# NNU-GISA/MetricSfM

Hardware: AMD Instinct MI355X
Metric: BA iterations/sec (higher is better)
Workload: dtype f64; 1 GPU; BASELINE config 3: 500 cameras / 200000 points / 1200000 observations, dense-Schur LM, Huber(1); reduced_system_order=3003, parallelism=points sharded over 1 rank(s), camera block all-reduced, collective=none (1 rank), successful_steps=2789, unsuccessful_steps=0

## Files before the change

metricsfm_amd/csrc/ba.hip:

```cpp
#include <algorithm>
#include <array>
#include <chrono>
#include <cmath>
#include <cstdlib>
#include <cstring>
#include <functional>

#include <rocprim/rocprim.hpp>

#include "ba_device.h"
#include "ba_partials.h"
#include "common.h"
#include "solve_riders.h"


#define PSTRIDE 80
#define CHUNK 1024
#define FTF_CHUNK 512
static int chunk_for(long total, int max_chunk) {
  const long c = 64 * ((total / 1024 + 63) / 64);
  return (int)std::max<long>(64, std::min<long>(max_chunk, c));
}
#define F_JCJC 0
#define F_JMJC 36
#define F_JMJM 54
#define F_JCR 63
#define F_JMR 69
#define F_TU 72
static_assert(PSTRIDE == MODELSUM_PSTRIDE && F_JMJM == MODELSUM_JMJM && F_JMR == MODELSUM_JMR, "solve_riders.h reads the FTF partials");

enum { S_COST = 0, S_MCC, S_DX2, S_X2, S_FAIL, S_XCOST, S_GMAX, S_RANK0 = 8, S_N = 64 };

struct BaPtrs {
  int A, AE, ncb, nmb, npb, NCR;
  const double *cam, *model, *pt;
  const double* rot;
  const int *o_cam, *o_model, *o_pt, *o_cb, *o_mb, *o_pb, *o_cpos, *o_pm;
  const double *o_x, *o_y, *o_w;
  double *lin_r, *lin_Jc, *lin_Jm;
  const double *scale_c, *scale_m, *scale_p;
  double huber;
};

__device__ __forceinline__ double linearize_core(const double (&pose)[6], const double (&rc)[4], const double (&cm)[3], const double (&X)[3], double ox,
                                                 double oy, double ow, const double (&sc)[6], const double (&sm)[3], const double (&sp)[3], double huber,
                                                 double& r0, double& r1, double (&jc)[12], double (&jm)[6], double (&jp)[6]) {
  double r[2], J[24];
  msfm_reproj(pose, rc, cm, X, ox, oy, ow, r, J);
  double rho0, rho1;
  msfm_huber(huber, r[0] * r[0] + r[1] * r[1], rho0, rho1);
  const double sq = sqrt(rho1);
  r0 = sq * r[0]; r1 = sq * r[1];
#pragma unroll
  for (int j = 0; j < 6; j++) {
    const double s = sq * sc[j];
    jc[j] = s * J[j];
    jc[6 + j] = s * J[12 + j];
  }
#pragma unroll
  for (int j = 0; j < 3; j++) {
    const double s = sq * sm[j];
    jm[j] = s * J[6 + j];
    jm[3 + j] = s * J[12 + 6 + j];
    const double spj = sq * sp[j];
    jp[j] = spj * J[9 + j];
    jp[3 + j] = spj * J[12 + 9 + j];
  }
  return 0.5 * rho0;
}
__device__ __forceinline__ double obs_linearize(const BaPtrs& P, int i, double& r0, double& r1, double (&jc)[12], double (&jm)[6], double (&jp)[6]) {
  const int c = P.o_cam[i], m = P.o_model[i], p = P.o_pt[i];
  const int cb = P.o_cb[i], mb = P.o_mb[i], pb = P.o_pb[i];
  double pose[6], rc[4], cm[3], X[3];
#pragma unroll
  for (int j = 0; j < 6; j++) pose[j] = P.cam[6 * (size_t)c + j];
#pragma unroll
  for (int j = 0; j < 4; j++) rc[j] = P.rot[4 * (size_t)c + j];
#pragma unroll
  for (int j = 0; j < 3; j++) { cm[j] = P.model[3 * (size_t)m + j]; X[j] = P.pt[3 * (size_t)p + j]; }
  const double ox = P.o_x[i], oy = P.o_y[i], ow = P.o_w[i];
  double r[2], J[24];
  msfm_reproj(pose, rc, cm, X, ox, oy, ow, r, J);
  __builtin_amdgcn_sched_barrier(0);
  double sc[6], sm[3], sp[3];
#pragma unroll
  for (int j = 0; j < 6; j++) sc[j] = cb >= 0 ? P.scale_c[6 * cb + j] : 0.0;
#pragma unroll
  for (int j = 0; j < 3; j++) { sm[j] = mb >= 0 ? P.scale_m[3 * mb + j] : 0.0; sp[j] = pb >= 0 ? P.scale_p[3 * (size_t)pb + j] : 0.0; }
  double rho0, rho1;
  msfm_huber(P.huber, r[0] * r[0] + r[1] * r[1], rho0, rho1);
  const double sq = sqrt(rho1);
  r0 = sq * r[0]; r1 = sq * r[1];
#pragma unroll
  for (int j = 0; j < 6; j++) {
    const double s = sq * sc[j];
    jc[j] = s * J[j];
    jc[6 + j] = s * J[12 + j];
  }
#pragma unroll
  for (int j = 0; j < 3; j++) {
    const double s = sq * sm[j];
    jm[j] = s * J[6 + j];
    jm[3 + j] = s * J[12 + 6 + j];
    const double spj = sq * sp[j];
    jp[j] = spj * J[9 + j];
    jp[3 + j] = spj * J[12 + 9 + j];
  }
  return 0.5 * rho0;
}
template <bool WRITE_JAC>
__device__ __forceinline__ void linearize_block(const BaPtrs& P, int i0, int blk, double* __restrict__ cost_partial, double* sh) {
  const int i = i0 + blk * 256 + threadIdx.x;
  double cost = 0.0;
  if (i < P.A) {
    if (WRITE_JAC) {
      double r0, r1, jc[12], jm[6], jp[6];
      cost = obs_linearize(P, i, r0, r1, jc, jm, jp);
      const size_t nt = (size_t)(P.A - P.AE), it = (size_t)(i - P.AE);
      P.lin_r[it] = r0;
      P.lin_r[nt + it] = r1;
#pragma unroll
      for (int j = 0; j < 12; j++) P.lin_Jc[(size_t)j * nt + it] = jc[j];
#pragma unroll
      for (int j = 0; j < 6; j++) P.lin_Jm[(size_t)j * nt + it] = jm[j];
    } else {
      const int c = P.o_cam[i], m = P.o_model[i], p = P.o_pt[i];
      double pose[6], rc[4], cm[3], X[3];
#pragma unroll
      for (int j = 0; j < 6; j++) pose[j] = P.cam[6 * (size_t)c + j];
#pragma unroll
      for (int j = 0; j < 4; j++) rc[j] = P.rot[4 * (size_t)c + j];
#pragma unroll
      for (int j = 0; j < 3; j++) { cm[j] = P.model[3 * (size_t)m + j]; X[j] = P.pt[3 * (size_t)p + j]; }
      double r[2];
      msfm_reproj(pose, rc, cm, X, P.o_x[i], P.o_y[i], P.o_w[i], r, nullptr);
      double rho0, rho1;
      msfm_huber(P.huber, r[0] * r[0] + r[1] * r[1], rho0, rho1);
      cost = 0.5 * rho0;
    }
  }
  const double t = block_sum256(cost, sh);
  if (threadIdx.x == 0) cost_partial[blk] = t;
}
template <bool WRITE_JAC>
__global__ __launch_bounds__(256) void k_linearize(BaPtrs P, int i0, double* __restrict__ cost_partial, const double* __restrict__ spec = nullptr) {
  __shared__ double sh[4];
  if (spec && spec[0] == 0.0) return;
  linearize_block<WRITE_JAC>(P, i0, blockIdx.x, cost_partial, sh);
}

__global__ __launch_bounds__(256) void k_rot_cache(int Nc, const double* __restrict__ cam, double* __restrict__ rot) {
  const int c = blockIdx.x * 256 + threadIdx.x;
  if (c < Nc) msfm_rot_prepare(cam + 6 * (size_t)c, rot + 4 * (size_t)c);
}

template <bool WRITE_JAC>
__device__ __forceinline__ void gps_block(int blk, int ncb, const int* __restrict__ cb_cam, const double* __restrict__ cam,
                                          const double* __restrict__ gps, double w, double huber,
                                          const double* __restrict__ scale_c, double* __restrict__ g_r,
                                          double* __restrict__ g_J, double* __restrict__ cost_partial, double* sh) {
  const int cb = blk * 256 + threadIdx.x;
  double cost = 0.0;
  if (cb < ncb) {
    const int c = cb_cam[cb];
    const double wz[3] = {w, w, w / 5.0};
    double r[3], J[3], s = 0.0;
#pragma unroll
    for (int k = 0; k < 3; k++) {
      const double d = cam[6 * (size_t)c + 3 + k] - gps[3 * (size_t)cb + k];
      r[k] = wz[k] * fabs(d);
      J[k] = wz[k] * (d < 0.0 ? -1.0 : 1.0);
      s += r[k] * r[k];
    }
    double rho0, rho1;
    msfm_huber(huber, s, rho0, rho1);
    cost = 0.5 * rho0;
    if (WRITE_JAC) {
      const double sq = sqrt(rho1);
#pragma unroll
      for (int k = 0; k < 3; k++) {
        g_r[3 * (size_t)cb + k] = sq * r[k];
        g_J[3 * (size_t)cb + k] = sq * J[k] * scale_c[6 * cb + 3 + k];
      }
    }
  }
  const double t = block_sum256(cost, sh);
  if (threadIdx.x == 0) cost_partial[blk] = t;
}
template <bool WRITE_JAC>
__global__ __launch_bounds__(256) void k_gps(int ncb, const int* __restrict__ cb_cam, const double* __restrict__ cam,
                                              const double* __restrict__ gps, double w, double huber,
                                              const double* __restrict__ scale_c, double* __restrict__ g_r,
                                              double* __restrict__ g_J, double* __restrict__ cost_partial, const double* __restrict__ spec = nullptr) {
  __shared__ double sh[4];
  if (spec && spec[0] == 0.0) return;
  gps_block<WRITE_JAC>(blockIdx.x, ncb, cb_cam, cam, gps, w, huber, scale_c, g_r, g_J, cost_partial, sh);
}

struct ReduceJobs {
  int count;
  struct { const double* p; int n; int slot; int is_max; } job[6];
  const int* fail;
  int fail_slot;
};
__global__ __launch_bounds__(1024) void k_reduce(ReduceJobs J, double* __restrict__ scal) {
  __shared__ double sh[16];
  const double* __restrict__ partial = J.job[blockIdx.x].p;
  const int n = J.job[blockIdx.x].n, slot = J.job[blockIdx.x].slot, is_max = J.job[blockIdx.x].is_max;
  double v0 = 0.0, v1 = 0.0, v2 = 0.0, v3 = 0.0;
  int i = threadIdx.x;
  for (; i + 3072 < n; i += 4096) {
    const double a = partial[i], b = partial[i + 1024], c = partial[i + 2048], d = partial[i + 3072];
    if (is_max) { v0 = fmax(v0, a); v1 = fmax(v1, b); v2 = fmax(v2, c); v3 = fmax(v3, d); }
    else { v0 += a; v1 += b; v2 += c; v3 += d; }
  }
  for (; i < n; i += 1024) v0 = is_max ? fmax(v0, partial[i]) : v0 + partial[i];
  double v = is_max ? fmax(fmax(v0, v1), fmax(v2, v3)) : (v0 + v1) + (v2 + v3);
  v = is_max ? wave_max(v) : wave_sum(v);
  if ((threadIdx.x & 63) == 0) sh[threadIdx.x >> 6] = v;
  __syncthreads();
  if (threadIdx.x == 0) {
    double t = sh[0];
// ... 901 lines not shown
#pragma unroll
    for (int k = 0; k < 9; k++) if (k == lane) v = -acc[k];
    if (rb == cbk && lead) {
      v += modelsum[12 * (size_t)rb + lane];
      if (a == c) { const double q = sqrt(diag_m[3 * rb + a] / radius); v += q * q; }
    }
    M[(size_t)(mo + 3 * rb + a) * ld + mo + 3 * cbk + c] = v;
  } else if (lane < 12 && rb == cbk) {
    const int a = lane - 9;
    double u = 0.0;
#pragma unroll
    for (int k = 9; k < 12; k++) if (k == lane) u = acc[k];
    M[(size_t)n * ld + mo + 3 * rb + a] = (lead ? modelsum[12 * (size_t)rb + 9 + a] : 0.0) - u;
  }
}

__device__ __forceinline__ void asm_rhs_cam(int i, int ncb, const double* __restrict__ camftf, const int* __restrict__ cb_off,
                                            double* __restrict__ M, int ld, int n, int lead) {
  if (i >= 6 * ncb) return;
  const int cb = i / 6, a = i % 6;
  const double* f = camftf + (size_t)cb * PSTRIDE;
  M[(size_t)n * ld + cb_off[cb] + a] = lead ? f[F_JCR + a] - f[F_TU + a] : 0.0;
}

struct AsmArgs {
  int n_cc, n_mc, n_mm, n_rhs, n_padcol;
  const int* padcol;
  const int* cc_fold_first;
  const uint8_t* cc_live;
  const double* cc_fold_partial;
  const int* mc_fold_range;
  const double* mc_fold_partial;
  const int *cc_row, *cc_col, *cc_first, *mc_row, *mc_col, *mc_first, *mm_row, *mm_col, *mm_first, *cb_mb, *cb_off;
  const double *cc_partial, *mc_partial, *mm_partial, *camftf, *diag_c, *modelsum, *diag_m;
  double radius;
  int ncb, mo, n, ld, lead;
  double* M;
};
__global__ __launch_bounds__(64) void k_asm_all(AsmArgs a) {
  int b = blockIdx.x;
  if (b < a.n_cc) {
    const int sub = (int)threadIdx.x / 18;
    asm_cc(b, sub, (int)threadIdx.x - 18 * sub, a.cc_row, a.cc_col, a.cc_first, a.cc_live, a.cc_partial, a.cc_fold_first, a.cc_fold_partial, a.camftf, a.diag_c, a.radius, a.cb_off, a.M, a.ld, a.lead);
    return;
  }
  b -= a.n_cc;
  if (b < a.n_mc) { asm_mc(b, a.mc_row, a.mc_col, a.mc_first, a.mc_partial, a.mc_fold_range, a.mc_fold_partial, a.camftf, a.cb_mb, a.cb_off, a.mo, a.M, a.ld, a.lead); return; }
  b -= a.n_mc;
  if (b < a.n_mm) { asm_mm(b, a.mm_row, a.mm_col, a.mm_first, a.mm_partial, a.modelsum, a.diag_m, a.radius, a.mo, a.n, a.M, a.ld, a.lead); return; }
  b -= a.n_mm;
  if (b < a.n_rhs) { asm_rhs_cam(b * 64 + (int)threadIdx.x, a.ncb, a.camftf, a.cb_off, a.M, a.ld, a.n, a.lead); return; }
  b -= a.n_rhs;
  const int i = b * 64 + (int)threadIdx.x;
  if (i < a.n_padcol) a.M[(size_t)a.padcol[i] * a.ld + a.padcol[i]] = 1.0;
}

__global__ void k_pad_diag(int npadcol, const int* __restrict__ padcol, double* __restrict__ M, int ld) {
  const int i = blockIdx.x * blockDim.x + threadIdx.x;
  if (i < npadcol) M[(size_t)padcol[i] * ld + padcol[i]] = 1.0;
}

__global__ __launch_bounds__(256) void k_copy3(size_t n0, const double* __restrict__ a0, double* __restrict__ b0, size_t n1,
                                               const double* __restrict__ a1, double* __restrict__ b1, size_t n2,
                                               const double* __restrict__ a2, double* __restrict__ b2) {
  const size_t i = (size_t)blockIdx.x * 256 + threadIdx.x;
  if (i < n0) b0[i] = a0[i];
  if (i < n1) b1[i] = a1[i];
  if (i < n2) b2[i] = a2[i];
}


__global__ void k_scale_scal(double* __restrict__ scal, int slot, double f) { scal[slot] *= f; }

__global__ __launch_bounds__(256) void k_update_params(int ncb, int nmb, const int* __restrict__ cb_cam, const int* __restrict__ mb_model,
                                                        const int* __restrict__ cb_off, int mo, const double* __restrict__ zsys,
                                                        const double* __restrict__ scale_c, const double* __restrict__ scale_m,
                                                        const double* __restrict__ cam, double* __restrict__ cam_c,
                                                        const double* __restrict__ model, double* __restrict__ model_c, double* __restrict__ z,
                                                        int* __restrict__ fail, double* __restrict__ dx2_partial, double* __restrict__ x2_partial,
                                                        double count_weight) {
  __shared__ double sh[4];
  const int i = blockIdx.x * 256 + threadIdx.x;
  double dx2 = 0.0, x2 = 0.0;
  if (i < 6 * ncb + 3 * nmb) {
    double zv, sc, xv;
    double* dst;
    if (i < 6 * ncb) {
      const int b = i / 6, a = i % 6;
      zv = zsys[cb_off[b] + a];
      sc = scale_c[i];
      const size_t k = (size_t)cb_cam[b] * 6 + a;
      xv = cam[k];
      dst = cam_c + k;
    } else {
      const int j = i - 6 * ncb, b = j / 3, a = j % 3;
      zv = zsys[mo + j];
      sc = scale_m[j];
      const size_t k = (size_t)mb_model[b] * 3 + a;
      xv = model[k];
      dst = model_c + k;
    }
    z[i] = zv;
    if (!isfinite(zv)) atomicOr(fail, 4);
    const double cand = xv + (-zv) * sc;
    *dst = cand;
    const double d = cand - xv;
    dx2 = d * d * count_weight;
    x2 = xv * xv * count_weight;
  }
  const double t1 = block_sum256(dx2, sh);
  const double t2 = block_sum256(x2, sh);
  if (threadIdx.x == 0) { dx2_partial[blockIdx.x] = t1; x2_partial[blockIdx.x] = t2; }
}
__global__ void k_col_map(int ncb, int nmb, const int* __restrict__ cb_cam, const int* __restrict__ mb_model, const int* __restrict__ cb_off,
                          int mo, int* __restrict__ col_param, int* __restrict__ col_slot) {
  const int i = blockIdx.x * 256 + threadIdx.x;
  if (i >= 6 * ncb + 3 * nmb) return;
  int col, slot;
  if (i < 6 * ncb) { const int b = i / 6, a = i % 6; col = cb_off[b] + a; slot = cb_cam[b] * 6 + a; }
  else { const int j = i - 6 * ncb, b = j / 3, a = j % 3; col = mo + j; slot = mb_model[b] * 3 + a; }
  col_param[col] = i;
  col_slot[col] = slot;
}
__device__ __forceinline__ void update_block_sums(int n, const double* __restrict__ dx2s, const double* __restrict__ x2s,
                                                  double* __restrict__ dx2_partial, double* __restrict__ x2_partial, double* sh) {
  const int i = blockIdx.x * 256 + threadIdx.x;
  double dx2 = 0.0, x2 = 0.0;
  if (i < n) { dx2 = dx2s[i]; x2 = x2s[i]; }
  const double t1 = block_sum256(dx2, sh);
  const double t2 = block_sum256(x2, sh);
  if (threadIdx.x == 0) { dx2_partial[blockIdx.x] = t1; x2_partial[blockIdx.x] = t2; }
}

struct BackPtrs {
  BaPtrs B;
  PtMap map;
  int npb, ncb;
  const int *pt_first, *pb_pt;
  const double *ptL, *z;
  double* pt_c;
  double* cm_Xc;
  int Nc;
  const double* cam_c;
  double* rot_c;
};
struct UpdateSums {
  int nbu, n;
  const double *dx2, *x2;
  double *dx2_partial, *x2_partial;
};

template <int LPP>
__device__ __forceinline__ void k_backsub_body(const BackPtrs& P, double* __restrict__ mcc_partial, double* __restrict__ dx2_partial,
                                               double* __restrict__ x2_partial, double* sh) {
  constexpr int GW = LPP ? LPP : 8;
  const int tid = threadIdx.x, sub = tid & (GW - 1);
  const int pb = ptmap_wg_first(P.map, blockIdx.x) + tid / GW;
  const bool act = pb < ptmap_wg_end(P.map, blockIdx.x);
  for (int c = blockIdx.x * 256 + tid; c < P.Nc; c += gridDim.x * 256) msfm_rot_prepare(P.cam_c + 6 * (size_t)c, P.rot_c + 4 * (size_t)c);
  int f = 0, l = 0;
  if (act) { f = P.pt_first[pb]; l = P.pt_first[pb + 1]; }
  double V00 = 0, V10 = 0, V11 = 0, V20 = 0, V21 = 0, V22 = 0, g0 = 0, g1 = 0, g2 = 0, h0 = 0, h1 = 0, h2 = 0, qr = 0, qq = 0;
  const int n_rounds = LPP ? 1 : (l - f + 7) >> 3;
  for (int rd = 0; rd < n_rounds; rd++) {
    const int i = f + GW * rd + sub;
    if (i < l) {
      double jp[6], r0, r1, q0, q1;
      {
        const int cb = P.B.o_cb[i], mb = P.B.o_mb[i];
        double jc[12], jm[6], zc[6], zm[3];
        obs_linearize(P.B, i, r0, r1, jc, jm, jp);
        __builtin_amdgcn_sched_barrier(0);
        const double* zcp = P.z + 6 * (cb >= 0 ? cb : 0);
        const double* zmp = P.z + 6 * P.ncb + 3 * (mb >= 0 ? mb : 0);
#pragma unroll
        for (int j = 0; j < 6; j++) zc[j] = zcp[j];
#pragma unroll
        for (int j = 0; j < 3; j++) zm[j] = zmp[j];
        q0 = 0.0; q1 = 0.0;
#pragma unroll
        for (int j = 0; j < 6; j++) { q0 -= jc[j] * zc[j]; q1 -= jc[6 + j] * zc[j]; }
#pragma unroll
        for (int j = 0; j < 3; j++) { q0 -= jm[j] * zm[j]; q1 -= jm[3 + j] * zm[j]; }
      }
      const double a0 = jp[0], a1 = jp[1], a2 = jp[2], b0 = jp[3], b1 = jp[4], b2 = jp[5];
      V00 += a0 * a0 + b0 * b0; V10 += a1 * a0 + b1 * b0; V11 += a1 * a1 + b1 * b1;
      V20 += a2 * a0 + b2 * b0; V21 += a2 * a1 + b2 * b1; V22 += a2 * a2 + b2 * b2;
      g0 += a0 * r0 + b0 * r1; g1 += a1 * r0 + b1 * r1; g2 += a2 * r0 + b2 * r1;
      h0 += a0 * q0 + b0 * q1; h1 += a1 * q0 + b1 * q1; h2 += a2 * q0 + b2 * q1;
      qr += q0 * r0 + q1 * r1;
      qq += q0 * q0 + q1 * q1;
    }
  }
  GROUP_SUM(V00) GROUP_SUM(V10) GROUP_SUM(V11) GROUP_SUM(V20) GROUP_SUM(V21) GROUP_SUM(V22)
  GROUP_SUM(g0) GROUP_SUM(g1) GROUP_SUM(g2) GROUP_SUM(h0) GROUP_SUM(h1) GROUP_SUM(h2) GROUP_SUM(qr) GROUP_SUM(qq)
  double mcc = 0.0, dx2 = 0.0, x2 = 0.0, cand0 = 0.0, cand1 = 0.0, cand2 = 0.0;
  if (act && sub == 0) {
    const double* L = P.ptL + 6 * (size_t)pb;
    const double i00 = L[0], l10 = L[1], i11 = L[2], l20 = L[3], l21 = L[4], i22 = L[5];
    double q0 = (g0 + h0) * i00;
    double q1 = ((g1 + h1) - l10 * q0) * i11;
    double q2 = ((g2 + h2) - l20 * q0 - l21 * q1) * i22;
    q2 = q2 * i22;
    q1 = (q1 - l21 * q2) * i11;
    q0 = (q0 - l10 * q1 - l20 * q2) * i00;
    const double s0 = -q0, s1 = -q1, s2 = -q2;
    const double* sc = P.B.scale_p + 3 * (size_t)pb;
    const size_t p = P.pb_pt[pb];
    const double x0 = P.B.pt[3 * p], x1 = P.B.pt[3 * p + 1], x2v = P.B.pt[3 * p + 2];
    const double c0 = x0 + s0 * sc[0], c1 = x1 + s1 * sc[1], c2 = x2v + s2 * sc[2];
    P.pt_c[3 * p] = c0; P.pt_c[3 * p + 1] = c1; P.pt_c[3 * p + 2] = c2;
    cand0 = c0; cand1 = c1; cand2 = c2;
    dx2 = (c0 - x0) * (c0 - x0) + (c1 - x1) * (c1 - x1) + (c2 - x2v) * (c2 - x2v);
    x2 = x0 * x0 + x1 * x1 + x2v * x2v;
    const double sVs = s0 * (V00 * s0 + 2.0 * (V10 * s1 + V20 * s2)) + s1 * (V11 * s1 + 2.0 * V21 * s2) + s2 * V22 * s2;
    mcc = -((s0 * g0 + s1 * g1 + s2 * g2) + qr + 0.5 * sVs + (s0 * h0 + s1 * h1 + s2 * h2) + 0.5 * qq);
  }
  cand0 = __shfl(cand0, 0, GW); cand1 = __shfl(cand1, 0, GW); cand2 = __shfl(cand2, 0, GW);
  for (int rd = 0; rd < n_rounds; rd++) {
    const int i = f + GW * rd + sub;
    if (i < l) {
      const int cp = P.B.o_cpos[i];
      if (cp >= 0) { double* xr = P.cm_Xc + 3 * (size_t)cp; xr[0] = cand0; xr[1] = cand1; xr[2] = cand2; }
    }
  }
  const double t0 = block_sum256(mcc, sh);
  const double t1 = block_sum256(dx2, sh);
  const double t2 = block_sum256(x2, sh);
  if (threadIdx.x == 0) { mcc_partial[blockIdx.x] = t0; dx2_partial[blockIdx.x] = t1; x2_partial[blockIdx.x] = t2; }
}
__global__ __launch_bounds__(256) __attribute__((amdgpu_waves_per_eu(3, 3))) void k_backsub(BackPtrs P, double* __restrict__ mcc_partial, double* __restrict__ dx2_partial,
                                                  double* __restrict__ x2_partial, UpdateSums U) {
  __shared__ double sh[4];
  const int lanes = ptmap_lanes(P.map, blockIdx.x);
  if (lanes == 4) k_backsub_body<4>(P, mcc_partial, dx2_partial, x2_partial, sh);
  else if (lanes == 8) k_backsub_body<8>(P, mcc_partial, dx2_partial, x2_partial, sh);
  else if (lanes == 16) k_backsub_body<16>(P, mcc_partial, dx2_partial, x2_partial, sh);
  else k_backsub_body<0>(P, mcc_partial, dx2_partial, x2_partial, sh);
  if ((int)blockIdx.x < U.nbu) update_block_sums(U.n, U.dx2, U.x2, U.dx2_partial, U.x2_partial, sh);
}

__device__ __forceinline__ void mcc_rest_block(int blk, int A, int AE, int ncb, const int* __restrict__ o_cb, const int* __restrict__ o_mb,
                                               const double* __restrict__ lin_r, const double* __restrict__ lin_Jc,
                                               const double* __restrict__ lin_Jm, const double* __restrict__ z, int has_gps,
                                               const double* __restrict__ g_r, const double* __restrict__ g_J,
                                               double* __restrict__ mcc_partial, double* sh) {
  const int t = blk * 256 + threadIdx.x;
  const int nrest = A - AE;
  double mcc = 0.0;
  if (t < nrest) {
    const int i = AE + t;
    const size_t As = (size_t)nrest, it = (size_t)t;
    double m0 = 0, m1 = 0;
    const int cb = o_cb[i], mb = o_mb[i];
    if (cb >= 0)
      for (int j = 0; j < 6; j++) { const double sj = -z[6 * cb + j]; m0 += lin_Jc[(size_t)j * As + it] * sj; m1 += lin_Jc[(size_t)(6 + j) * As + it] * sj; }
    if (mb >= 0)
      for (int j = 0; j < 3; j++) { const double sj = -z[6 * ncb + 3 * mb + j]; m0 += lin_Jm[(size_t)j * As + it] * sj; m1 += lin_Jm[(size_t)(3 + j) * As + it] * sj; }
    mcc -= m0 * (lin_r[it] + m0 / 2.0) + m1 * (lin_r[As + it] + m1 / 2.0);
  } else if (has_gps && t < nrest + ncb) {
    const int cb = t - nrest;
    for (int k = 0; k < 3; k++) {
      const double m = g_J[3 * (size_t)cb + k] * (-z[6 * cb + 3 + k]);
      mcc -= m * (g_r[3 * (size_t)cb + k] + m / 2.0);
    }
  }
  const double s = block_sum256(mcc, sh);
  if (threadIdx.x == 0) mcc_partial[blk] = s;
}

struct TailArgs {
  int n_zero; double* M; int ld; ZeroMap Z;
  int n_mcc, n_cost, n_gps;
  int A, AE, ncb; const int *o_cb, *o_mb; const double *lin_r, *lin_Jc, *lin_Jm, *z; int has_gps; const double *g_r, *g_J; double* mcc_partial;
  BaPtrs P; double* cost_partial;
  const int* cb_cam; const double *cam_c, *gps; double gps_weight, huber; const double* scale_c; double *g_r_w, *g_J_w;
};
__global__ __launch_bounds__(256) void k_tail(TailArgs a) {
  __shared__ double sh[4];
  int b = blockIdx.x;
  if (b < a.n_zero) { zero_tile_body(b, a.M, a.ld, a.Z); return; }
  b -= a.n_zero;
  if (b < a.n_mcc) { mcc_rest_block(b, a.A, a.AE, a.ncb, a.o_cb, a.o_mb, a.lin_r, a.lin_Jc, a.lin_Jm, a.z, a.has_gps, a.g_r, a.g_J, a.mcc_partial, sh); return; }
  b -= a.n_mcc;
  if (b < a.n_cost) { linearize_block<false>(a.P, 0, b, a.cost_partial, sh); return; }
  b -= a.n_cost;
  gps_block<false>(b, a.ncb, a.cb_cam, a.cam_c, a.gps, a.gps_weight, a.huber, a.scale_c, a.g_r_w, a.g_J_w, a.cost_partial + a.n_cost, sh);
}

__global__ void k_zero_int(int* p) { *p = 0; }
enum { LM_NONE = 0, LM_INVALID, LM_PARAM_TOL, LM_FUNC_TOL, LM_ACCEPT, LM_REJECT };
enum { H_SEQ = 16, H_CODE = 17, H_RADIUS = 18 };
struct LmDecide {
  int on;
  int fresh;
  double x_cost, radius;
  double min_relative_decrease, parameter_tolerance, function_tolerance, max_radius, min_radius;
};
__device__ __forceinline__ double cube_rn(double t) {
  const double h = t * t, l = fma(t, t, -h);
  const double p = h * t, e = fma(h, t, -p);
  return p + fma(l, t, e);
}
__global__ __launch_bounds__(64) void k_publish_scalars(const double* __restrict__ scal, double* h_scal, unsigned long long seq, int* fail, LmDecide D,
                                                        double* __restrict__ spec) {
  const int lane = threadIdx.x;
  if (lane < 16) __hip_atomic_store(&h_scal[lane], scal[lane], __ATOMIC_RELAXED, __HIP_MEMORY_SCOPE_SYSTEM);
  if (lane == 0) {
    int code = LM_NONE;
    double rnew = D.radius;
    if (D.on) {
      const double mcc = scal[S_MCC], cand = scal[S_COST], dx2 = scal[S_DX2], x2 = scal[S_X2];
      const double xc = D.fresh ? scal[S_XCOST] : D.x_cost;
      const bool solved = (int)scal[S_FAIL] == 0;
      if (!(solved && mcc > 0.0)) code = LM_INVALID;
      else if (sqrt(dx2) <= D.parameter_tolerance * (sqrt(x2) + D.parameter_tolerance)) code = LM_PARAM_TOL;
      else if (fabs(xc - cand) <= D.function_tolerance * xc) code = LM_FUNC_TOL;
      else {
        const double rho = (xc - cand) / mcc;
        if (rho > D.min_relative_decrease) {
          code = LM_ACCEPT;
          rnew = D.radius / fmax(1.0 / 3.0, 1.0 - cube_rn(2.0 * rho - 1.0));
          rnew = fmin(D.max_radius, rnew);
        } else code = LM_REJECT;
      }
    }
    spec[0] = (code == LM_ACCEPT && rnew > D.min_radius) ? 1.0 : 0.0;
    spec[1] = rnew;
    __hip_atomic_store(&h_scal[H_CODE], (double)code, __ATOMIC_RELAXED, __HIP_MEMORY_SCOPE_SYSTEM);
    __hip_atomic_store(&h_scal[H_RADIUS], rnew, __ATOMIC_RELAXED, __HIP_MEMORY_SCOPE_SYSTEM);
  }
  __threadfence_system();
  if (lane == 0) {
    __hip_atomic_store(reinterpret_cast<unsigned long long*>(h_scal + H_SEQ), seq, __ATOMIC_RELEASE, __HIP_MEMORY_SCOPE_SYSTEM);
    if (fail) *fail = 0;
  }
}
__global__ void k_fill(int n, double v, double* __restrict__ p) {
  const int i = blockIdx.x * 256 + threadIdx.x;
  if (i < n) p[i] = v;
}

template <bool PACK>
__global__ __launch_bounds__(256) void k_pack_blocks(int nblk, const int* __restrict__ u_row, const int* __restrict__ u_col,
                                                      const int* __restrict__ cb_off, double* __restrict__ M, int ld,
                                                      double* __restrict__ pack) {
  const int e = blockIdx.x * 256 + threadIdx.x;
  if (e >= nblk * 36) return;
  const int b = e / 36, t = e - 36 * b;
  const size_t at = (size_t)(cb_off[u_row[b]] + t / 6) * ld + cb_off[u_col[b]] + t % 6;
  if (PACK) pack[e] = M[at];
  else M[at] = pack[e];
}

struct FoldTables {
  bool on = false;
  bool all = false;
  int n_live = 0;
  DevBuf<int> live_chunk;
  int n_wg = 0, n_slots = 0, n_entries = 0, n_pass = 0;
  DevBuf<int> wg_fold, wg_pass_first, slot_rank, blk_range;
  DevBuf<uint8_t> blk_live;
  DevBuf<FoldPass> pass;
  DevBuf<unsigned> stream;
  DevBuf<double> partial;
  bool mc_on = false, mc_all = false;
  int n_diag = 0, mc_n_live = 0;
  long long mc_entries_folded = 0;
  DevBuf<int> mc_range, mc_live_chunk;
  DevBuf<double> mc_partial;
};

struct PairJobs {
  int n_pairs = 0, n_chunks = 0, n_blocks = 0;
  DevBuf<int> pa, pb, ch_start, ch_end, blk_row, blk_col, blk_chunk_first;
  DevBuf<double> partial;
  std::vector<int> h_row, h_col;
};

struct msfm_ba {
  msfm_ctx* ctx = nullptr;
  msfm_env env;
  int world_at_create = 1;
  double setup_ms = 0;
  int Nc = 0, Nm = 0, Np = 0;
  int ncb = 0, nmb = 0, npb = 0, nred = 0, npad = 0;
  PtMap map = {0, 0, 0, 0, 0, 0, 0};
  int n_short4 = 0;
  int nsys = 0, mo = 0, n_padcol = 0;
  msfm_chol_plan plan;
  int A = 0, AE = 0, NCR = 0, NPM = 0;
// ... 2627 lines not shown
```

metricsfm_amd/csrc/ba_device.h:

```cpp
#pragma once
#include <hip/hip_runtime.h>

__device__ __forceinline__ void msfm_rot_prepare(const double* __restrict__ pose, double* __restrict__ rc) {
  const double a0 = pose[0], a1 = pose[1], a2 = pose[2];
  const double theta2 = a0 * a0 + a1 * a1 + a2 * a2;
  double s = 0.0, c = 1.0, ti = 0.0, flag = 0.0;
  if (theta2 > 2.220446049250313e-16) {
    const double theta = sqrt(theta2);
    sincos(theta, &s, &c);
    ti = 1.0 / theta;
    flag = 1.0;
  }
  rc[0] = flag; rc[1] = s; rc[2] = c; rc[3] = ti;
}

__device__ __forceinline__ void msfm_reproj(const double* __restrict__ pose, const double* __restrict__ rc, const double* __restrict__ cam,
                                            const double* __restrict__ xyz, double ox, double oy, double weight,
                                            double* r, double* J) {
  const double a0 = pose[0], a1 = pose[1], a2 = pose[2];
  const double X0 = xyz[0], X1 = xyz[1], X2 = xyz[2];
  double p0, p1, p2;
  double dpdw[9];
  double R[9];
  if (rc[0] != 0.0) {
    const double s = rc[1], c = rc[2], ti = rc[3];
    const double w0 = a0 * ti, w1 = a1 * ti, w2 = a2 * ti;
    const double wx0 = w1 * X2 - w2 * X1, wx1 = w2 * X0 - w0 * X2, wx2 = w0 * X1 - w1 * X0;
    const double wdx = w0 * X0 + w1 * X1 + w2 * X2;
    const double omc = 1.0 - c;
    const double tmp = wdx * omc;
    p0 = X0 * c + wx0 * s + w0 * tmp;
    p1 = X1 * c + wx1 * s + w1 * tmp;
    p2 = X2 * c + wx2 * s + w2 * tmp;
    if (J) {
      const double w[3] = {w0, w1, w2};
      const double wx[3] = {wx0, wx1, wx2};
      const double Xv[3] = {X0, X1, X2};
#pragma unroll
      for (int j = 0; j < 3; j++) {
        double dw[3];
#pragma unroll
        for (int i = 0; i < 3; i++) dw[i] = ((i == j ? 1.0 : 0.0) - w[i] * w[j]) * ti;
        const double dwx[3] = {dw[1] * X2 - dw[2] * X1, dw[2] * X0 - dw[0] * X2, dw[0] * X1 - dw[1] * X0};
        const double dwdx = dw[0] * X0 + dw[1] * X1 + dw[2] * X2;
        const double dc = -s * w[j], ds = c * w[j];
        const double dtmp = dwdx * omc - wdx * dc;
#pragma unroll
        for (int i = 0; i < 3; i++) dpdw[i * 3 + j] = Xv[i] * dc + dwx[i] * s + wx[i] * ds + dw[i] * tmp + w[i] * dtmp;
      }
      R[0] = c + w0 * w0 * omc;      R[1] = w0 * w1 * omc - w2 * s; R[2] = w1 * s + w0 * w2 * omc;
      R[3] = w2 * s + w0 * w1 * omc; R[4] = c + w1 * w1 * omc;      R[5] = -w0 * s + w1 * w2 * omc;
      R[6] = -w1 * s + w0 * w2 * omc; R[7] = w0 * s + w1 * w2 * omc; R[8] = c + w2 * w2 * omc;
    }
  } else {
    p0 = X0 + (a1 * X2 - a2 * X1);
    p1 = X1 + (a2 * X0 - a0 * X2);
    p2 = X2 + (a0 * X1 - a1 * X0);
    if (J) {
      dpdw[0] = 0;   dpdw[1] = X2;  dpdw[2] = -X1;
      dpdw[3] = -X2; dpdw[4] = 0;   dpdw[5] = X0;
      dpdw[6] = X1;  dpdw[7] = -X0; dpdw[8] = 0;
      R[0] = 1;   R[1] = -a2; R[2] = a1;
      R[3] = a2;  R[4] = 1;   R[5] = -a0;
      R[6] = -a1; R[7] = a0;  R[8] = 1;
    }
  }
  p0 += pose[3]; p1 += pose[4]; p2 += pose[5];
  const double iz = 1.0 / p2;
  const double xp = J ? p0 * iz : p0 / p2, yp = J ? p1 * iz : p1 / p2;
  const double f = cam[0], l1 = cam[1], l2 = cam[2];
  const double r2 = xp * xp + yp * yp;
  const double dist = 1.0 + r2 * (l1 + l2 * r2);
  r[0] = weight * (f * dist * xp - ox);
  r[1] = weight * (f * dist * yp - oy);
  if (!J) return;
  const double dd = l1 + 2.0 * l2 * r2;
  const double uxp = f * (dist + 2.0 * xp * xp * dd), uyp = f * 2.0 * xp * yp * dd;
  const double vxp = uyp, vyp = f * (dist + 2.0 * yp * yp * dd);
  const double up[3] = {uxp * iz, uyp * iz, -(uxp * xp + uyp * yp) * iz};
  const double vp[3] = {vxp * iz, vyp * iz, -(vxp * xp + vyp * yp) * iz};
#pragma unroll
  for (int j = 0; j < 3; j++) {
    J[j] = weight * (up[0] * dpdw[j] + up[1] * dpdw[3 + j] + up[2] * dpdw[6 + j]);
    J[12 + j] = weight * (vp[0] * dpdw[j] + vp[1] * dpdw[3 + j] + vp[2] * dpdw[6 + j]);
    J[3 + j] = weight * up[j];
    J[12 + 3 + j] = weight * vp[j];
    J[9 + j] = weight * (up[0] * R[j] + up[1] * R[3 + j] + up[2] * R[6 + j]);
    J[12 + 9 + j] = weight * (vp[0] * R[j] + vp[1] * R[3 + j] + vp[2] * R[6 + j]);
  }
  J[6] = weight * dist * xp;        J[12 + 6] = weight * dist * yp;
  J[7] = weight * f * r2 * xp;      J[12 + 7] = weight * f * r2 * yp;
  J[8] = weight * f * r2 * r2 * xp; J[12 + 8] = weight * f * r2 * r2 * yp;
}

__device__ __forceinline__ void msfm_huber(double a, double s, double& rho0, double& rho1) {
  const double b = a * a;
  if (s > b) {
    const double r = sqrt(s);
    rho0 = 2.0 * a * r - b;
    rho1 = fmax(2.2250738585072014e-308, a / r);
  } else {
    rho0 = s;
    rho1 = 1.0;
  }
}

template <int CTRL>
__device__ __forceinline__ double dpp_f64(double v) {
  const int lo = __builtin_amdgcn_update_dpp(0, __double2loint(v), CTRL, 0xf, 0xf, false);
  const int hi = __builtin_amdgcn_update_dpp(0, __double2hiint(v), CTRL, 0xf, 0xf, false);
  return __hiloint2double(hi, lo);
}
#define MSFM_DPP_XOR1 0xB1
#define MSFM_DPP_XOR2 0x4E
#define MSFM_DPP_ROR8 0x128
#define MSFM_DPP_HALF_MIRROR 0x141
__device__ __forceinline__ int dpp_xor4_b32(int x) {
  const int t = __builtin_amdgcn_update_dpp(0, x, 0x104, 0xf, 0x5, false);
  return __builtin_amdgcn_update_dpp(t, x, 0x114, 0xf, 0xa, false);
}
__device__ __forceinline__ double dpp_xor4_f64(double v) {
  return __hiloint2double(dpp_xor4_b32(__double2hiint(v)), dpp_xor4_b32(__double2loint(v)));
}
__device__ __forceinline__ void swap16_f64(double v, double& a, double& b) {
  const unsigned lo = __double2loint(v), hi = __double2hiint(v);
  const auto l = __builtin_amdgcn_permlane16_swap(lo, lo, false, false);
  const auto h = __builtin_amdgcn_permlane16_swap(hi, hi, false, false);
  a = __hiloint2double(h[0], l[0]);
  b = __hiloint2double(h[1], l[1]);
}
__device__ __forceinline__ void swap32_f64(double v, double& a, double& b) {
  const unsigned lo = __double2loint(v), hi = __double2hiint(v);
  const auto l = __builtin_amdgcn_permlane32_swap(lo, lo, false, false);
  const auto h = __builtin_amdgcn_permlane32_swap(hi, hi, false, false);
  a = __hiloint2double(h[0], l[0]);
  b = __hiloint2double(h[1], l[1]);
}
__device__ __forceinline__ double wave_sum(double v) {
  double a, b;
  swap32_f64(v, a, b); v = a + b;
  swap16_f64(v, a, b); v = a + b;
  v += dpp_f64<MSFM_DPP_ROR8>(v);
  v += dpp_xor4_f64(v);
  v += dpp_f64<MSFM_DPP_XOR2>(v);
  v += dpp_f64<MSFM_DPP_XOR1>(v);
  return v;
}
__device__ __forceinline__ double wave_max(double v) {
  double a, b;
  swap32_f64(v, a, b); v = fmax(a, b);
  swap16_f64(v, a, b); v = fmax(a, b);
  v = fmax(v, dpp_f64<MSFM_DPP_ROR8>(v));
  v = fmax(v, dpp_xor4_f64(v));
  v = fmax(v, dpp_f64<MSFM_DPP_XOR2>(v));
  v = fmax(v, dpp_f64<MSFM_DPP_XOR1>(v));
  return v;
}
template <int D>
__device__ __forceinline__ double partner_f64(double t) {
  if constexpr (D == 8) return dpp_f64<MSFM_DPP_ROR8>(t);
  else if constexpr (D == 4) return dpp_xor4_f64(t);
  else if constexpr (D == 2) return dpp_f64<MSFM_DPP_XOR2>(t);
  else return dpp_f64<MSFM_DPP_XOR1>(t);
}
template <int D, int n, int N>
__device__ __forceinline__ void reduce_scatter_step(double (&v)[N], int lane) {
  constexpr int h = (n + 1) / 2;
  const bool low = (lane & D) == 0;
#pragma unroll
  for (int j = 0; j < h; j++) {
    const double a = v[j], b = (h + j < n) ? v[h + j] : 0.0;
    if constexpr (D == 32) { double x, y; const unsigned al = __double2loint(a), ah = __double2hiint(a), bl = __double2loint(b), bh = __double2hiint(b);
      const auto l = __builtin_amdgcn_permlane32_swap(al, bl, false, false); const auto hh = __builtin_amdgcn_permlane32_swap(ah, bh, false, false);
      x = __hiloint2double(hh[0], l[0]); y = __hiloint2double(hh[1], l[1]); v[j] = x + y;
    } else if constexpr (D == 16) { double x, y; const unsigned al = __double2loint(a), ah = __double2hiint(a), bl = __double2loint(b), bh = __double2hiint(b);
      const auto l = __builtin_amdgcn_permlane16_swap(al, bl, false, false); const auto hh = __builtin_amdgcn_permlane16_swap(ah, bh, false, false);
      x = __hiloint2double(hh[0], l[0]); y = __hiloint2double(hh[1], l[1]); v[j] = x + y;
    } else {
      const double t = low ? b : a;
      const double mine = low ? a : b;
      v[j] = mine + partner_f64<D>(t);
    }
  }
}
template <int N>
__device__ __forceinline__ void wave_reduce_scatter(double (&v)[N], int lane, double& val, int& idx) {
  constexpr int n1 = (N + 1) / 2, n2 = (n1 + 1) / 2, n3 = (n2 + 1) / 2, n4 = (n3 + 1) / 2, n5 = (n4 + 1) / 2;
  static_assert(N <= 64 && (n5 + 1) / 2 == 1, "at most 64 values");
  reduce_scatter_step<32, N>(v, lane);
  reduce_scatter_step<16, n1>(v, lane);
  reduce_scatter_step<8, n2>(v, lane);
  reduce_scatter_step<4, n3>(v, lane);
  reduce_scatter_step<2, n4>(v, lane);
  reduce_scatter_step<1, n5>(v, lane);
  val = v[0];
  int lo = 0, nv = N, n = N;
#pragma unroll
  for (int d = 32; d >= 1; d >>= 1) {
    const int h = (n + 1) / 2;
    if (lane & d) { lo += h; nv = max(0, nv - h); } else nv = min(nv, h);
    n = h;
  }
  idx = nv > 0 ? lo : -1;
}

__device__ __forceinline__ double block_sum256(double v, double* sh ) {
  v = wave_sum(v);
  const int w = threadIdx.x >> 6;
  if ((threadIdx.x & 63) == 0) sh[w] = v;
  __syncthreads();
  double t = 0.0;
  if (threadIdx.x == 0) t = (sh[0] + sh[1]) + (sh[2] + sh[3]);
  __syncthreads();
  return t;
}
__device__ __forceinline__ double block_max256(double v, double* sh) {
  v = wave_max(v);
  const int w = threadIdx.x >> 6;
  if ((threadIdx.x & 63) == 0) sh[w] = v;
  __syncthreads();
  double t = 0.0;
  if (threadIdx.x == 0) t = fmax(fmax(sh[0], sh[1]), fmax(sh[2], sh[3]));
  __syncthreads();
  return t;
}

struct PtMap {
  int nQ, nS, nL, nX;
  int wQ, wS, wL;
};
__host__ __device__ inline int ptmap_lanes(const PtMap& m, int w) { return w < m.wQ ? 4 : w < m.wQ + m.wS ? 8 : w < m.wQ + m.wS + m.wL ? 16 : 0; }
__host__ __device__ inline int ptmap_wg_points(int lanes) { return lanes ? 256 / lanes : 32; }
__host__ __device__ inline int ptmap_wg_first(const PtMap& m, int w) {
  if (w < m.wQ) return 64 * w;
  w -= m.wQ;
  if (w < m.wS) return m.nQ + 32 * w;
  w -= m.wS;
  if (w < m.wL) return m.nQ + m.nS + 16 * w;
  return m.nQ + m.nS + m.nL + 32 * (w - m.wL);
}
__host__ __device__ inline int ptmap_wg_end(const PtMap& m, int w) {
  const int e = ptmap_wg_first(m, w) + ptmap_wg_points(ptmap_lanes(m, w));
  const int cap = w < m.wQ ? m.nQ : w < m.wQ + m.wS ? m.nQ + m.nS : w < m.wQ + m.wS + m.wL ? m.nQ + m.nS + m.nL : m.nQ + m.nS + m.nL + m.nX;
  return e < cap ? e : cap;
}
__host__ __device__ inline int ptmap_wg_of(const PtMap& m, int pb) {
  if (pb < m.nQ) return pb >> 6;
  pb -= m.nQ;
  if (pb < m.nS) return m.wQ + (pb >> 5);
  pb -= m.nS;
  if (pb < m.nL) return m.wQ + m.wS + (pb >> 4);
  return m.wQ + m.wS + m.wL + ((pb - m.nL) >> 5);
}
#define PTMAP_CLASSES 4
__host__ __device__ inline int ptmap_class(int rows) { return rows <= 4 ? 0 : rows <= 8 ? 1 : rows <= 16 ? 2 : 3; }
inline bool ptmap_use_lanes4(int npb, long min_points) { return npb > (min_points < 0 ? 32L * 3 * 256 : min_points); }
// ... 6 lines not shown
```

Measured before the change: 1267 iterations/s.

## Compute backsub J*z via directional derivative instead of full Jacobian

Adds a specialized backsub row routine that computes the camera/model Jacobian-times-update product as a directional derivative of the projection, and only forms the 3x2 point Jacobian explicitly instead of building the full 24-entry Jacobian. Point coordinates, scales and the Cholesky factor are hoisted out of the observation loop. For the variable-length path, the 14 per-lane accumulators move into a shared-memory array, and the occupancy target is raised from 3 to 4 waves per EU to relieve register pressure. The derivation must be algebraically exact for all rotation branches, and the shared-memory accumulators add LDS traffic and raise per-block LDS use.

```diff
diff --git a/metricsfm_amd/csrc/ba.hip b/metricsfm_amd/csrc/ba.hip
--- a/metricsfm_amd/csrc/ba.hip
+++ b/metricsfm_amd/csrc/ba.hip
@@ -42,32 +42,6 @@
   double huber;
 };
 
-__device__ __forceinline__ double linearize_core(const double (&pose)[6], const double (&rc)[4], const double (&cm)[3], const double (&X)[3], double ox,
-                                                 double oy, double ow, const double (&sc)[6], const double (&sm)[3], const double (&sp)[3], double huber,
-                                                 double& r0, double& r1, double (&jc)[12], double (&jm)[6], double (&jp)[6]) {
-  double r[2], J[24];
-  msfm_reproj(pose, rc, cm, X, ox, oy, ow, r, J);
-  double rho0, rho1;
-  msfm_huber(huber, r[0] * r[0] + r[1] * r[1], rho0, rho1);
-  const double sq = sqrt(rho1);
-  r0 = sq * r[0]; r1 = sq * r[1];
-#pragma unroll
-  for (int j = 0; j < 6; j++) {
-    const double s = sq * sc[j];
-    jc[j] = s * J[j];
-    jc[6 + j] = s * J[12 + j];
-  }
-#pragma unroll
-  for (int j = 0; j < 3; j++) {
-    const double s = sq * sm[j];
-    jm[j] = s * J[6 + j];
-    jm[3 + j] = s * J[12 + 6 + j];
-    const double spj = sq * sp[j];
-    jp[j] = spj * J[9 + j];
-    jp[3 + j] = spj * J[12 + 9 + j];
-  }
-  return 0.5 * rho0;
-}
 __device__ __forceinline__ double obs_linearize(const BaPtrs& P, int i, double& r0, double& r1, double (&jc)[12], double (&jm)[6], double (&jp)[6]) {
   const int c = P.o_cam[i], m = P.o_model[i], p = P.o_pt[i];
   const int cb = P.o_cb[i], mb = P.o_mb[i], pb = P.o_pb[i];
@@ -1275,7 +1249,7 @@
 
 template <int LPP>
 __device__ __forceinline__ void k_backsub_body(const BackPtrs& P, double* __restrict__ mcc_partial, double* __restrict__ dx2_partial,
-                                               double* __restrict__ x2_partial, double* sh) {
+                                               double* __restrict__ x2_partial, double* sh, double* xacc ) {
   constexpr int GW = LPP ? LPP : 8;
   const int tid = threadIdx.x, sub = tid & (GW - 1);
   const int pb = ptmap_wg_first(P.map, blockIdx.x) + tid / GW;
@@ -1283,44 +1257,62 @@
   for (int c = blockIdx.x * 256 + tid; c < P.Nc; c += gridDim.x * 256) msfm_rot_prepare(P.cam_c + 6 * (size_t)c, P.rot_c + 4 * (size_t)c);
   int f = 0, l = 0;
   if (act) { f = P.pt_first[pb]; l = P.pt_first[pb + 1]; }
+  size_t p = 0;
+  double X[3] = {0, 0, 0}, sp[3] = {0, 0, 0}, Lf[6] = {0, 0, 0, 0, 0, 0};
+  if (act) {
+    p = P.pb_pt[pb];
+#pragma unroll
+    for (int j = 0; j < 3; j++) { X[j] = P.B.pt[3 * p + j]; sp[j] = P.B.scale_p[3 * (size_t)pb + j]; }
+  }
   double V00 = 0, V10 = 0, V11 = 0, V20 = 0, V21 = 0, V22 = 0, g0 = 0, g1 = 0, g2 = 0, h0 = 0, h1 = 0, h2 = 0, qr = 0, qq = 0;
+  if constexpr (LPP == 0) {
+#pragma unroll
+    for (int k = 0; k < 14; k++) xacc[k * 256 + tid] = 0.0;
+  }
   const int n_rounds = LPP ? 1 : (l - f + 7) >> 3;
   for (int rd = 0; rd < n_rounds; rd++) {
     const int i = f + GW * rd + sub;
     if (i < l) {
+      const int c = P.B.o_cam[i], m = P.B.o_model[i], cb = P.B.o_cb[i], mb = P.B.o_mb[i];
+      const double ox = P.B.o_x[i], oy = P.B.o_y[i], ow = P.B.o_w[i];
+      const double* zcp = P.z + 6 * (cb >= 0 ? cb : 0);
+      const double* zmp = P.z + 6 * P.ncb + 3 * (mb >= 0 ? mb : 0);
+      double pose[6], rc[4], cm[3], sc[6], sm[3], zc[6], zm[3];
+#pragma unroll
+      for (int j = 0; j < 6; j++) { pose[j] = P.B.cam[6 * (size_t)c + j]; sc[j] = cb >= 0 ? P.B.scale_c[6 * cb + j] : 0.0; zc[j] = zcp[j]; }
+#pragma unroll
+      for (int j = 0; j < 4; j++) rc[j] = P.B.rot[4 * (size_t)c + j];
+#pragma unroll
+      for (int j = 0; j < 3; j++) { cm[j] = P.B.model[3 * (size_t)m + j]; sm[j] = mb >= 0 ? P.B.scale_m[3 * mb + j] : 0.0; zm[j] = zmp[j]; }
       double jp[6], r0, r1, q0, q1;
-      {
-        const int cb = P.B.o_cb[i], mb = P.B.o_mb[i];
-        double jc[12], jm[6], zc[6], zm[3];
-        obs_linearize(P.B, i, r0, r1, jc, jm, jp);
-        __builtin_amdgcn_sched_barrier(0);
-        const double* zcp = P.z + 6 * (cb >= 0 ? cb : 0);
-        const double* zmp = P.z + 6 * P.ncb + 3 * (mb >= 0 ? mb : 0);
-#pragma unroll
-        for (int j = 0; j < 6; j++) zc[j] = zcp[j];
-#pragma unroll
-        for (int j = 0; j < 3; j++) zm[j] = zmp[j];
-        q0 = 0.0; q1 = 0.0;
-#pragma unroll
-        for (int j = 0; j < 6; j++) { q0 -= jc[j] * zc[j]; q1 -= jc[6 + j] * zc[j]; }
-#pragma unroll
-        for (int j = 0; j < 3; j++) { q0 -= jm[j] * zm[j]; q1 -= jm[3 + j] * zm[j]; }
+      msfm_backsub_row(pose, rc, cm, X, ox, oy, ow, sc, sm, sp, zc, zm, P.B.huber, r0, r1, jp, q0, q1);
+      const double a0 = jp[0], a1 = jp[1], a2 = jp[2], b0 = jp[3], b1 = jp[4], b2 = jp[5];
+      const double t[14] = {a0 * a0 + b0 * b0, a1 * a0 + b1 * b0, a1 * a1 + b1 * b1, a2 * a0 + b2 * b0, a2 * a1 + b2 * b1, a2 * a2 + b2 * b2,
+                            a0 * r0 + b0 * r1, a1 * r0 + b1 * r1, a2 * r0 + b2 * r1, a0 * q0 + b0 * q1, a1 * q0 + b1 * q1, a2 * q0 + b2 * q1,
+                            q0 * r0 + q1 * r1, q0 * q0 + q1 * q1};
+      if constexpr (LPP == 0) {
+#pragma unroll
+        for (int k = 0; k < 14; k++) xacc[k * 256 + tid] += t[k];
+      } else {
+        V00 += t[0]; V10 += t[1]; V11 += t[2]; V20 += t[3]; V21 += t[4]; V22 += t[5]; g0 += t[6]; g1 += t[7]; g2 += t[8];
+        h0 += t[9]; h1 += t[10]; h2 += t[11]; qr += t[12]; qq += t[13];
       }
-      const double a0 = jp[0], a1 = jp[1], a2 = jp[2], b0 = jp[3], b1 = jp[4], b2 = jp[5];
-      V00 += a0 * a0 + b0 * b0; V10 += a1 * a0 + b1 * b0; V11 += a1 * a1 + b1 * b1;
-      V20 += a2 * a0 + b2 * b0; V21 += a2 * a1 + b2 * b1; V22 += a2 * a2 + b2 * b2;
-      g0 += a0 * r0 + b0 * r1; g1 += a1 * r0 + b1 * r1; g2 += a2 * r0 + b2 * r1;
-      h0 += a0 * q0 + b0 * q1; h1 += a1 * q0 + b1 * q1; h2 += a2 * q0 + b2 * q1;
-      qr += q0 * r0 + q1 * r1;
-      qq += q0 * q0 + q1 * q1;
-    }
+    }
+  }
+  if constexpr (LPP == 0) {
+    V00 = xacc[tid]; V10 = xacc[256 + tid]; V11 = xacc[2 * 256 + tid]; V20 = xacc[3 * 256 + tid]; V21 = xacc[4 * 256 + tid]; V22 = xacc[5 * 256 + tid];
+    g0 = xacc[6 * 256 + tid]; g1 = xacc[7 * 256 + tid]; g2 = xacc[8 * 256 + tid]; h0 = xacc[9 * 256 + tid]; h1 = xacc[10 * 256 + tid]; h2 = xacc[11 * 256 + tid];
+    qr = xacc[12 * 256 + tid]; qq = xacc[13 * 256 + tid];
+  }
+  if (act && sub == 0) {
+#pragma unroll
+    for (int j = 0; j < 6; j++) Lf[j] = P.ptL[6 * (size_t)pb + j];
   }
   GROUP_SUM(V00) GROUP_SUM(V10) GROUP_SUM(V11) GROUP_SUM(V20) GROUP_SUM(V21) GROUP_SUM(V22)
   GROUP_SUM(g0) GROUP_SUM(g1) GROUP_SUM(g2) GROUP_SUM(h0) GROUP_SUM(h1) GROUP_SUM(h2) GROUP_SUM(qr) GROUP_SUM(qq)
   double mcc = 0.0, dx2 = 0.0, x2 = 0.0, cand0 = 0.0, cand1 = 0.0, cand2 = 0.0;
   if (act && sub == 0) {
-    const double* L = P.ptL + 6 * (size_t)pb;
-    const double i00 = L[0], l10 = L[1], i11 = L[2], l20 = L[3], l21 = L[4], i22 = L[5];
+    const double i00 = Lf[0], l10 = Lf[1], i11 = Lf[2], l20 = Lf[3], l21 = Lf[4], i22 = Lf[5];
     double q0 = (g0 + h0) * i00;
     double q1 = ((g1 + h1) - l10 * q0) * i11;
     double q2 = ((g2 + h2) - l20 * q0 - l21 * q1) * i22;
@@ -1328,10 +1320,8 @@
     q1 = (q1 - l21 * q2) * i11;
     q0 = (q0 - l10 * q1 - l20 * q2) * i00;
     const double s0 = -q0, s1 = -q1, s2 = -q2;
-    const double* sc = P.B.scale_p + 3 * (size_t)pb;
-    const size_t p = P.pb_pt[pb];
-    const double x0 = P.B.pt[3 * p], x1 = P.B.pt[3 * p + 1], x2v = P.B.pt[3 * p + 2];
-    const double c0 = x0 + s0 * sc[0], c1 = x1 + s1 * sc[1], c2 = x2v + s2 * sc[2];
+    const double x0 = X[0], x1 = X[1], x2v = X[2];
+    const double c0 = x0 + s0 * sp[0], c1 = x1 + s1 * sp[1], c2 = x2v + s2 * sp[2];
     P.pt_c[3 * p] = c0; P.pt_c[3 * p + 1] = c1; P.pt_c[3 * p + 2] = c2;
     cand0 = c0; cand1 = c1; cand2 = c2;
     dx2 = (c0 - x0) * (c0 - x0) + (c1 - x1) * (c1 - x1) + (c2 - x2v) * (c2 - x2v);
@@ -1352,14 +1342,15 @@
   const double t2 = block_sum256(x2, sh);
   if (threadIdx.x == 0) { mcc_partial[blockIdx.x] = t0; dx2_partial[blockIdx.x] = t1; x2_partial[blockIdx.x] = t2; }
 }
-__global__ __launch_bounds__(256) __attribute__((amdgpu_waves_per_eu(3, 3))) void k_backsub(BackPtrs P, double* __restrict__ mcc_partial, double* __restrict__ dx2_partial,
+__global__ __launch_bounds__(256) __attribute__((amdgpu_waves_per_eu(4, 4))) void k_backsub(BackPtrs P, double* __restrict__ mcc_partial, double* __restrict__ dx2_partial,
                                                   double* __restrict__ x2_partial, UpdateSums U) {
   __shared__ double sh[4];
+  __shared__ double xacc[14 * 256];
   const int lanes = ptmap_lanes(P.map, blockIdx.x);
-  if (lanes == 4) k_backsub_body<4>(P, mcc_partial, dx2_partial, x2_partial, sh);
-  else if (lanes == 8) k_backsub_body<8>(P, mcc_partial, dx2_partial, x2_partial, sh);
-  else if (lanes == 16) k_backsub_body<16>(P, mcc_partial, dx2_partial, x2_partial, sh);
-  else k_backsub_body<0>(P, mcc_partial, dx2_partial, x2_partial, sh);
+  if (lanes == 4) k_backsub_body<4>(P, mcc_partial, dx2_partial, x2_partial, sh, xacc);
+  else if (lanes == 8) k_backsub_body<8>(P, mcc_partial, dx2_partial, x2_partial, sh, xacc);
+  else if (lanes == 16) k_backsub_body<16>(P, mcc_partial, dx2_partial, x2_partial, sh, xacc);
+  else k_backsub_body<0>(P, mcc_partial, dx2_partial, x2_partial, sh, xacc);
   if ((int)blockIdx.x < U.nbu) update_block_sums(U.n, U.dx2, U.x2, U.dx2_partial, U.x2_partial, sh);
 }
 
diff --git a/metricsfm_amd/csrc/ba_device.h b/metricsfm_amd/csrc/ba_device.h
--- a/metricsfm_amd/csrc/ba_device.h
+++ b/metricsfm_amd/csrc/ba_device.h
@@ -1,7 +1,7 @@
 #pragma once
 #include <hip/hip_runtime.h>
 
-__device__ __forceinline__ void msfm_rot_prepare(const double* __restrict__ pose, double* __restrict__ rc) {
+__host__ __device__ __forceinline__ void msfm_rot_prepare(const double* __restrict__ pose, double* __restrict__ rc) {
   const double a0 = pose[0], a1 = pose[1], a2 = pose[2];
   const double theta2 = a0 * a0 + a1 * a1 + a2 * a2;
   double s = 0.0, c = 1.0, ti = 0.0, flag = 0.0;
@@ -14,9 +14,9 @@
   rc[0] = flag; rc[1] = s; rc[2] = c; rc[3] = ti;
 }
 
-__device__ __forceinline__ void msfm_reproj(const double* __restrict__ pose, const double* __restrict__ rc, const double* __restrict__ cam,
-                                            const double* __restrict__ xyz, double ox, double oy, double weight,
-                                            double* r, double* J) {
+__host__ __device__ __forceinline__ void msfm_reproj(const double* __restrict__ pose, const double* __restrict__ rc, const double* __restrict__ cam,
+                                                     const double* __restrict__ xyz, double ox, double oy, double weight,
+                                                     double* r, double* J) {
   const double a0 = pose[0], a1 = pose[1], a2 = pose[2];
   const double X0 = xyz[0], X1 = xyz[1], X2 = xyz[2];
   double p0, p1, p2;
@@ -93,7 +93,7 @@
   J[8] = weight * f * r2 * r2 * xp; J[12 + 8] = weight * f * r2 * r2 * yp;
 }
 
-__device__ __forceinline__ void msfm_huber(double a, double s, double& rho0, double& rho1) {
+__host__ __device__ __forceinline__ void msfm_huber(double a, double s, double& rho0, double& rho1) {
   const double b = a * a;
   if (s > b) {
     const double r = sqrt(s);
@@ -102,6 +102,103 @@
   } else {
     rho0 = s;
     rho1 = 1.0;
+  }
+}
+
+__host__ __device__ __forceinline__ double linearize_core(const double (&pose)[6], const double (&rc)[4], const double (&cm)[3], const double (&X)[3], double ox,
+                                                          double oy, double ow, const double (&sc)[6], const double (&sm)[3], const double (&sp)[3], double huber,
+                                                          double& r0, double& r1, double (&jc)[12], double (&jm)[6], double (&jp)[6]) {
+  double r[2], J[24];
+  msfm_reproj(pose, rc, cm, X, ox, oy, ow, r, J);
+  double rho0, rho1;
+  msfm_huber(huber, r[0] * r[0] + r[1] * r[1], rho0, rho1);
+  const double sq = sqrt(rho1);
+  r0 = sq * r[0]; r1 = sq * r[1];
+#pragma unroll
+  for (int j = 0; j < 6; j++) {
+    const double s = sq * sc[j];
+    jc[j] = s * J[j];
+    jc[6 + j] = s * J[12 + j];
+  }
+#pragma unroll
+  for (int j = 0; j < 3; j++) {
+    const double s = sq * sm[j];
+    jm[j] = s * J[6 + j];
+    jm[3 + j] = s * J[12 + 6 + j];
+    const double spj = sq * sp[j];
+    jp[j] = spj * J[9 + j];
+    jp[3 + j] = spj * J[12 + 9 + j];
+  }
+  return 0.5 * rho0;
+}
+
+__host__ __device__ __forceinline__ void msfm_backsub_row(const double (&pose)[6], const double (&rc)[4], const double (&cm)[3], const double (&X)[3],
+                                                          double ox, double oy, double weight, const double (&sc)[6], const double (&sm)[3],
+                                                          const double (&sp)[3], const double (&zc)[6], const double (&zm)[3], double huber,
+                                                          double& r0, double& r1, double (&jp)[6], double& q0, double& q1) {
+  const double a0 = pose[0], a1 = pose[1], a2 = pose[2];
+  const double X0 = X[0], X1 = X[1], X2 = X[2];
+  const double da0 = -(sc[0] * zc[0]), da1 = -(sc[1] * zc[1]), da2 = -(sc[2] * zc[2]);
+  const double dt0 = -(sc[3] * zc[3]), dt1 = -(sc[4] * zc[4]), dt2 = -(sc[5] * zc[5]);
+  const double df = -(sm[0] * zm[0]), dl1 = -(sm[1] * zm[1]), dl2 = -(sm[2] * zm[2]);
+  const double cx0 = da1 * X2 - da2 * X1, cx1 = da2 * X0 - da0 * X2, cx2 = da0 * X1 - da1 * X0;
+  double p0, p1, p2, dp0, dp1, dp2;
+  double w0, w1, w2, s, c, omc;
+  if (rc[0] != 0.0) {
+    s = rc[1]; c = rc[2];
+    const double ti = rc[3];
+    w0 = a0 * ti; w1 = a1 * ti; w2 = a2 * ti;
+    const double wx0 = w1 * X2 - w2 * X1, wx1 = w2 * X0 - w0 * X2, wx2 = w0 * X1 - w1 * X0;
+    const double wdx = w0 * X0 + w1 * X1 + w2 * X2;
+    omc = 1.0 - c;
+    const double tmp = wdx * omc;
+    p0 = X0 * c + wx0 * s + w0 * tmp;
+    p1 = X1 * c + wx1 * s + w1 * tmp;
+    p2 = X2 * c + wx2 * s + w2 * tmp;
+    const double swdx = s * wdx, k2 = 2.0 * tmp;
+    const double v0 = (c * wx0 - s * X0 + swdx * w0) - ti * (s * wx0 + k2 * w0);
+    const double v1 = (c * wx1 - s * X1 + swdx * w1) - ti * (s * wx1 + k2 * w1);
+    const double v2 = (c * wx2 - s * X2 + swdx * w2) - ti * (s * wx2 + k2 * w2);
+    const double wda = w0 * da0 + w1 * da1 + w2 * da2;
+    const double xda = X0 * da0 + X1 * da1 + X2 * da2;
+    dp0 = v0 * wda + ti * (s * cx0 + omc * (xda * w0 + wdx * da0)) + dt0;
+    dp1 = v1 * wda + ti * (s * cx1 + omc * (xda * w1 + wdx * da1)) + dt1;
+    dp2 = v2 * wda + ti * (s * cx2 + omc * (xda * w2 + wdx * da2)) + dt2;
+  } else {
+    p0 = X0 + (a1 * X2 - a2 * X1);
+    p1 = X1 + (a2 * X0 - a0 * X2);
+    p2 = X2 + (a0 * X1 - a1 * X0);
+    dp0 = cx0 + dt0; dp1 = cx1 + dt1; dp2 = cx2 + dt2;
+    w0 = a0; w1 = a1; w2 = a2; s = 1.0; c = 1.0; omc = 0.0;
+  }
+  p0 += pose[3]; p1 += pose[4]; p2 += pose[5];
+  const double iz = 1.0 / p2;
+  const double xp = p0 * iz, yp = p1 * iz;
+  const double f = cm[0], l1 = cm[1], l2 = cm[2];
+  const double r2 = xp * xp + yp * yp;
+  const double dist = 1.0 + r2 * (l1 + l2 * r2);
+  const double ru = weight * (f * dist * xp - ox);
+  const double rv = weight * (f * dist * yp - oy);
+  double rho0, rho1;
+  msfm_huber(huber, ru * ru + rv * rv, rho0, rho1);
+  const double sq = sqrt(rho1);
+  r0 = sq * ru; r1 = sq * rv;
+  const double dd = l1 + 2.0 * l2 * r2;
+  const double uxp = f * (dist + 2.0 * xp * xp * dd), uyp = f * 2.0 * xp * yp * dd, vyp = f * (dist + 2.0 * yp * yp * dd);
+  const double dxp = (dp0 - xp * dp2) * iz, dyp = (dp1 - yp * dp2) * iz;
+  const double m = dist * df + f * r2 * (dl1 + r2 * dl2);
+  const double ws = weight * sq;
+  q0 = ws * (uxp * dxp + uyp * dyp + xp * m);
+  q1 = ws * (uyp * dxp + vyp * dyp + yp * m);
+  const double wi = ws * iz;
+  const double g[2][3] = {{uxp * wi, uyp * wi, -(uxp * xp + uyp * yp) * wi}, {uyp * wi, vyp * wi, -(uyp * xp + vyp * yp) * wi}};
+#pragma unroll
+  for (int k = 0; k < 2; k++) {
+    const double g0 = g[k][0], g1 = g[k][1], g2 = g[k][2];
+    const double gw = omc * (g0 * w0 + g1 * w1 + g2 * w2);
+    jp[3 * k + 0] = sp[0] * (c * g0 + s * (g1 * w2 - g2 * w1) + gw * w0);
+    jp[3 * k + 1] = sp[1] * (c * g1 + s * (g2 * w0 - g0 * w2) + gw * w1);
+    jp[3 * k + 2] = sp[2] * (c * g2 + s * (g0 * w1 - g1 * w0) + gw * w2);
   }
 }
 
```

Measured after the change: 1292 iterations/s (median of 6 runs). 1.02x the previous value.
